# zabaras/deep-turbulence

Measured on AMD Instinct MI355X. Metric: flow-field samples/sec (fwd+log-det+bwd), 64x256x256x4; optimizer step: HipAdam (one-launch Adam, same update as torch.optim.Adam), higher is better.
Workload: dtype f32; 1 GPU; tmglow M: sample()+logdet+backward+Adam, out 256x256x4, L=4, K=16, batch 64/GPU; global_batch=64, parallelism=dp1, world_size_observed=1, rank0_device=AMD Radeon Graphics cuda:0, mix_precision=f32, launch=eager

## Files before the change

### deep-turbulence_amd/csrc/tmg_wino.hip

```cpp
#include "tmg_common.h"
#include <stdlib.h>
#include <type_traits>

struct WinoP {
    TmgSeg in[TMG_MAX_IN_SEG];
    int nseg;
    int B, Hin, Win;
    int Cin, Cin_pad, Cout, Npad;
    const float* U;
    const float* bias;
    int relu_in, pad_rep;
    TmgOSeg out[TMG_MAX_OUT_SEG];
    int tiles_x, tiles_y, ntiles;
    int nchunks;
};

__global__ void wino_pack_kernel(const float* __restrict__ w, float* __restrict__ U, int Cout, int Cin, int K, int N, int Kpad, int Npad, int mode) {
    const size_t total = (size_t)Kpad * Npad;
    for (size_t i = blockIdx.x * (size_t)blockDim.x + threadIdx.x; i < total; i += (size_t)gridDim.x * blockDim.x) {
        const int c16 = i & 15;
        size_t r = i >> 4;
        const int n = r % Npad;
        const int kb = r / Npad;
        const int k = kb * 16 + c16;
        float g[3][3];
#pragma unroll
        for (int a = 0; a < 3; ++a)
#pragma unroll
            for (int b = 0; b < 3; ++b) {
                float v = 0.f;
                if (k < K && n < N) v = mode == 0 ? w[((size_t)n * Cin + k) * 9 + a * 3 + b] : w[((size_t)k * Cin + n) * 9 + (2 - a) * 3 + (2 - b)];
                g[a][b] = v;
            }
        float t[4][3];
#pragma unroll
        for (int b = 0; b < 3; ++b) {
            t[0][b] = g[0][b];
            t[1][b] = 0.5f * (g[0][b] + g[1][b] + g[2][b]);
            t[2][b] = 0.5f * (g[0][b] - g[1][b] + g[2][b]);
            t[3][b] = g[2][b];
        }
#pragma unroll
        for (int a = 0; a < 4; ++a) {
            const float u0 = t[a][0], u1 = 0.5f * (t[a][0] + t[a][1] + t[a][2]), u2 = 0.5f * (t[a][0] - t[a][1] + t[a][2]), u3 = t[a][2];
            const size_t plane = (size_t)Kpad * Npad;
            U[(size_t)(a * 4 + 0) * plane + i] = u0;
            U[(size_t)(a * 4 + 1) * plane + i] = u1;
            U[(size_t)(a * 4 + 2) * plane + i] = u2;
            U[(size_t)(a * 4 + 3) * plane + i] = u3;
        }
    }
}

extern "C" int tmg_conv_wino_pack(const void* w, void* U, int64_t Cout, int64_t Cin, int64_t mode, int64_t nvalid, hipStream_t st) {
    const int K = mode == 0 ? (int)Cin : (int)Cout;
    const int N = mode == 0 ? (int)Cout : (int)(nvalid > 0 && nvalid < Cin ? nvalid : Cin);
    const int Kpad = (K + 15) & ~15, Npad = (N + 15) & ~15;
    const size_t total = (size_t)Kpad * Npad;
    const int blocks = (int)((total + 255) / 256 < 2048 ? (total + 255) / 256 : 2048);
    hipLaunchKernelGGL(wino_pack_kernel, dim3(blocks), dim3(256), 0, st, (const float*)w, (float*)U, (int)Cout, (int)Cin, K, N, Kpad, Npad, (int)mode);
    TMG_CHECK_LAUNCH();
    return 0;
}

constexpr int NT = 512;
constexpr int TH = 8, TW = 16, PH = TH + 2, PW = TW + 2, PP = PH * PW;
constexpr int KC = 32, CS = KC + 8;
constexpr int RAWW = PP * CS;
constexpr int UPI = (PP * (KC / 4) + NT - 1) / NT;
constexpr int VS = KC + 8;
constexpr int VPL = 32 * VS;

#define TMG_WN_TILE(T_)                                                                                               \
    int t_ = (T_);                                                                                                    \
    const int tx_ = t_ % p.tiles_x; t_ /= p.tiles_x;                                                                  \
    const int ty_ = t_ % p.tiles_y;                                                                                   \
    const int b_ = t_ / p.tiles_y;
#define TMG_WN_CURSORS                                                                                                \
    const int G = gridDim.x;                                                                                          \
    const int nmine = (int)blockIdx.x < p.ntiles ? (p.ntiles - (int)blockIdx.x + G - 1) / G : 0;                      \
    const int nchunks = p.nchunks, nst = nmine * nchunks;
#define TMG_WN_PATCH_TABLE                                                                                            \
    const int pc4 = tid & 7, ppix0 = tid >> 3;                                                                        \
    unsigned pyx[UPI];                                                                                                \
    _Pragma("unroll") for (int u = 0; u < UPI; ++u) {                                                                 \
        const int pix = min(ppix0 + u * 64, PP - 1);                                                                  \
        const int py = pix / PW, px = pix - py * PW;                                                                  \
        pyx[u] = ((unsigned)py << 16) | (unsigned)px;                                                                 \
    }                                                                                                                 \
    float4 pv[UPI];
#define TMG_WN_COMMIT                                                                                                 \
    if (k >= -1 && k + 1 < nst) {                                                                                     \
        float* rb_ = lds + ((k + 1) & 1) * RAWW;                                                                      \
        _Pragma("unroll") for (int u = 0; u < UPI; ++u) {                                                             \
            if (ppix0 + u * 64 < PP) {                                                                                \
                float4 v = pv[u];                                                                                     \
                if (p.relu_in) v = tmg_relu4(v); \
                *reinterpret_cast<float4*>(rb_ + (ppix0 + u * 64) * CS + 4 * pc4) = v;                                \
            }                                                                                                         \
        }                                                                                                             \
    }
#define TMG_WN_ISSUE_HEAD                                                                                             \
    TMG_WN_TILE(ti)                                                                                                   \
    const int iy0 = ty_ * TH - 1, ix0 = tx_ * TW - 1;                                                                 \
    TMG_PICK_IN_CHANNEL(p, ci * KC + 4 * pc4, true, tmg_zero_page, tptr, tss)
#define TMG_WN_ISSUE_TAIL if (++ci == nchunks) { ci = 0; ti += G; }
#define TMG_WN_PIXEL(U_)                                                                                              \
    const int iy = iy0 + (int)(pyx[U_] >> 16), ix = ix0 + (int)(pyx[U_] & 0xffffu);                                   \
    const int iyc = min(max(iy, 0), p.Hin - 1), ixc = min(max(ix, 0), p.Win - 1);                                     \
    const bool oob = !p.pad_rep && (iy != iyc || ix != ixc);
#define TMG_WN_TBV const unsigned tbv = (unsigned)b_ * (unsigned)(p.Hin * p.Win);
#define TMG_WN_PXI (tbv + (unsigned)iyc * (unsigned)p.Win + (unsigned)ixc)
#define TMG_WN_DEAD(U_) (oob || ppix0 + U_ * 64 >= PP)
#define TMG_WN_ISSUE(LOAD_)                                                                                           \
    if (k + 2 < nst) {                                                                                                \
        TMG_WN_ISSUE_HEAD                                                                                             \
        TMG_WN_TBV                                                                                                    \
        _Pragma("unroll") for (int u = 0; u < UPI; ++u) {                                                             \
            TMG_WN_PIXEL(u)                                                                                           \
            const float* a_ = TMG_WN_DEAD(u) ? tmg_zero_page : tptr + (size_t)TMG_WN_PXI * (unsigned)tss;             \
            LOAD_(pv[u], a_)                                                                                          \
        }                                                                                                             \
        TMG_WN_ISSUE_TAIL                                                                                             \
    }
#define TMG_WN_LD(D_, A_) D_ = *reinterpret_cast<const float4*>(A_);
#define TMG_WN_LD_NT(D_, A_)                                                                                          \
    {                                                                                                                 \
        const f32x4 nt_ = __builtin_nontemporal_load(reinterpret_cast<const f32x4*>(A_));                             \
        D_ = make_float4(nt_[0], nt_[1], nt_[2], nt_[3]);                                                             \
    }
#define TMG_W4(OP, A_, B_) make_float4(A_.x OP B_.x, A_.y OP B_.y, A_.z OP B_.z, A_.w OP B_.w)
#define TMG_WN_Y_RESET                                                                                                \
    _Pragma("unroll") for (int o = 0; o < 4; ++o) _Pragma("unroll") for (int m = 0; m < 2; ++m)                       \
        _Pragma("unroll") for (int n = 0; n < NPW; ++n) Y[o][m][n] = bvr[n];
#define TMG_WN_BIAS_Y                                                                                                 \
    f32x4 bvr[NPW];                                                                                                   \
    _Pragma("unroll") for (int n = 0; n < NPW; ++n) {                                                                 \
        const int n0 = (ntile0 + n) * 16 + 4 * q;                                                                     \
        const float* bp = (p.bias != nullptr && ntile0 + n < ntt && n0 < p.Cout) ? p.bias + n0 : tmg_zero_page;       \
        const float4 b4 = *reinterpret_cast<const float4*>(bp);                                                       \
        bvr[n] = (f32x4){b4.x, b4.y, b4.z, b4.w};                                                                     \
    }                                                                                                                 \
    f32x4 Y[4][2][NPW];                                                                                               \
    TMG_WN_Y_RESET
#define TMG_WN_EPILOGUE(LI_, Q_, STORE_)                                                                              \
    {                                                                                                                 \
        _Pragma("unroll") for (int m = 0; m < 2; ++m) {                                                               \
            const int wt = 16 * m + LI_;                                                                              \
            const int oyb = ty_ * TH + 2 * (wt >> 3), oxb = tx_ * TW + 2 * (wt & 7);                                  \
            _Pragma("unroll") for (int n = 0; n < NPW; ++n) {                                                         \
                const int n0 = (ntile0 + n) * 16 + 4 * Q_;                                                            \
                if (ntile0 + n < ntt && n0 < p.Cout) {                                                                \
                    int nl = n0;                                                                                      \
                    TMG_PICK_OSEG(p.out, nl, optr, ostride, ooff)                                                     \
                    _Pragma("unroll") for (int o = 0; o < 4; ++o) {                                                   \
                        const int oy = oyb + (o >> 1), ox = oxb + (o & 1);                                            \
                        if (oy < p.Hin && ox < p.Win) {                                                               \
                            const unsigned opx = ((unsigned)b_ * (unsigned)p.Hin + (unsigned)oy) * (unsigned)p.Win + (unsigned)ox; \
                            STORE_(Y[o][m][n], optr + (size_t)opx * (unsigned)ostride + ooff + nl)                    \
                        }                                                                                             \
                    }                                                                                                 \
                }                                                                                                     \
            }                                                                                                         \
        }                                                                                                             \
        TMG_WN_Y_RESET                                                                                                \
        cm = 0; tm += G;                                                                                              \
// ... 735 lines not shown
            if (cm + 1 == nchunks) {
#pragma unroll
                for (int e = 0; e < 2; ++e)
#pragma unroll
                    for (int m = 0; m < 2; ++m)
#pragma unroll
                        for (int n = 0; n < NTN; ++n) {
                            *reinterpret_cast<float4*>(Mb + ((pos0 + e) * 32 + 16 * m + li) * NC + 16 * n + 4 * q) =
                                make_float4(acc[e][m][n][0], acc[e][m][n][1], acc[e][m][n][2], acc[e][m][n][3]);
                            acc[e][m][n] = (f32x4){0.f, 0.f, 0.f, 0.f};
                        }
                __syncthreads();
                TMG_WN_TILE(tm)
                static_assert(32 * QN <= NT, "one epilogue item per thread");
                for (int it = tid; it < 32 * QN; it += NT) {
                    const int wt = it / QN, c4 = it - wt * QN;
                    const int n0 = 4 * c4;
                    if (n0 >= p.Cout) continue;
                    const float* mp_ = Mb + wt * NC + n0;
                    float4 z[2][4];
#pragma unroll
                    for (int nu = 0; nu < 4; ++nu) {
                        const float4 m0 = *reinterpret_cast<const float4*>(mp_ + (0 * 4 + nu) * 32 * NC);
                        const float4 m1 = *reinterpret_cast<const float4*>(mp_ + (1 * 4 + nu) * 32 * NC);
                        const float4 m2 = *reinterpret_cast<const float4*>(mp_ + (2 * 4 + nu) * 32 * NC);
                        const float4 m3 = *reinterpret_cast<const float4*>(mp_ + (3 * 4 + nu) * 32 * NC);
                        z[0][nu] = make_float4(m0.x + m1.x + m2.x, m0.y + m1.y + m2.y, m0.z + m1.z + m2.z, m0.w + m1.w + m2.w);
                        z[1][nu] = make_float4(m1.x - m2.x - m3.x, m1.y - m2.y - m3.y, m1.z - m2.z - m3.z, m1.w - m2.w - m3.w);
                    }
                    const float4 bv = bvq;
                    int nl = n0;
                    TMG_PICK_OSEG(p.out, nl, optr, ostride, ooff)
#pragma unroll
                    for (int oy = 0; oy < 2; ++oy)
#pragma unroll
                        for (int ox = 0; ox < 2; ++ox) {
                            const float4 za = z[oy][0], zb = z[oy][1], zc = z[oy][2], zd = z[oy][3];
                            float4 y = ox == 0 ? make_float4(za.x + zb.x + zc.x, za.y + zb.y + zc.y, za.z + zb.z + zc.z, za.w + zb.w + zc.w)
                                               : make_float4(zb.x - zc.x - zd.x, zb.y - zc.y - zd.y, zb.z - zc.z - zd.z, zb.w - zc.w - zd.w);
                            y.x += bv.x; y.y += bv.y; y.z += bv.z; y.w += bv.w;
                            if (p.relu_out) y = tmg_relu4(y);
                            const int py = ty_ * TH + 2 * (wt >> 3) + oy, px = tx_ * TW + 2 * (wt & 7) + ox;
                            if (py < p.Hin && px < p.Win)
                                *reinterpret_cast<float4*>(optr + (size_t)(((unsigned)b_ * (unsigned)p.Hin + (unsigned)py) * (unsigned)p.Win + (unsigned)px) * (unsigned)ostride + ooff + nl) = y;
                        }
                }
                cm = 0; tm += G;
            } else {
                ++cm;
            }
        }
        __syncthreads();
    }
#undef TMG_WN_STAGE
#undef TMG_WN_LOADG
}

template <int NTN>
static int launch_wino_nn(const WinoNP& p, int G, hipStream_t st, int64_t* plan) {
    const size_t lds_bytes = (size_t)(2 * 180 * 40 + 16 * 32 * (NTN * 16 + (NTN < 3 ? 4 : 0))) * sizeof(float);
    if (plan) { fill_wino_fwd_plan(plan, 3, NTN, p, G, 1, lds_bytes); return 0; }
    TMG_LDS_OPTIN((&wino_nn_kernel<NTN>));
    TmgProf prof(TMG_PROF_WINO, 2.0 * p.B * p.Hin * p.Win * (double)p.Cout * p.Cin * 9, st);
    hipLaunchKernelGGL((wino_nn_kernel<NTN>), dim3(G), dim3(512), lds_bytes, st, p);
    TMG_CHECK_LAUNCH();
    return 0;
}

static int wino_narrow_impl(const void* const* in_ptrs, const int64_t* in_desc, int64_t nseg, const void* U, const void* bias,
                            void* const* out_ptrs, const int64_t* out_desc, int64_t nout, const int64_t* dims, hipStream_t st, int64_t* plan) {
    WinoNP p;
    const int rc = wino_fwd_setup(p, in_ptrs, in_desc, nseg, U, bias, out_ptrs, out_desc, nout, dims, 16, true);
    if (rc != 1) return rc;
    p.relu_out = (int)dims[7];
    const int G = tmg_persistent_grid(1, p.ntiles);
    switch (p.Npad >> 4) {
        case 1: return launch_wino_nn<1>(p, G, st, plan);
        case 2: return launch_wino_nn<2>(p, G, st, plan);
        default: return launch_wino_nn<3>(p, G, st, plan);
    }
}

extern "C" int tmg_conv_wino_narrow(const void* const* in_ptrs, const int64_t* in_desc, int64_t nseg, const void* U, const void* bias,
                                    void* const* out_ptrs, const int64_t* out_desc, int64_t nout, const int64_t* dims, hipStream_t st) {
    return wino_narrow_impl(in_ptrs, in_desc, nseg, U, bias, out_ptrs, out_desc, nout, dims, st, nullptr);
}

extern "C" int tmg_conv_wino_narrow_plan(const void* const* in_ptrs, const int64_t* in_desc, int64_t nseg, const void* U, const void* bias,
                                         void* const* out_ptrs, const int64_t* out_desc, int64_t nout, const int64_t* dims, hipStream_t st,
                                         int64_t* plan) {
    if (!plan) return -3;
    for (int i = 0; i < TMG_WINO_FWD_PLAN_N; ++i) plan[i] = -1;
    return wino_narrow_impl(in_ptrs, in_desc, nseg, U, bias, out_ptrs, out_desc, nout, dims, st, plan);
}

struct WinoWP {
    TmgSeg in[TMG_MAX_IN_SEG];
    int nseg;
    int B, Hin, Win;
    int Cin, Cout;
    int relu_in, pad_rep;
    const float* dy; int dy_stride, dy_off;
    float* ws;
    int want_bias;
    const long long* gtab;
    int bpg, dy_goff;
    int tiles_x, tiles_y, ntiles;
};

template <int CIT, int NCO, bool DB>
__global__ __launch_bounds__(512, 1) void wino_wgrad_kernel(WinoWP p) {
    extern __shared__ __attribute__((aligned(16))) float lds[];
// ... 420 lines not shown
```

### deep-turbulence_amd/tmg_hip.py

```python
import ctypes
import os
import weakref
import subprocess
import sys

import torch

_HERE = os.path.dirname(os.path.abspath(__file__))
LIB_PATH = os.path.join(_HERE, "libtmglow_hip.so")
CSRC = os.path.join(_HERE, "csrc")
SOURCES = ["tmg_conv.hip", "tmg_pointwise.hip", "tmg_physics.hip", "tmg_mix16.hip", "tmg_coupling.hip", "tmg_wino.hip", "tmg_thin.hip", "tmg_glue.hip", "tmg_ensemble.hip", "tmg_spectrum.hip", "tmg_scores.hip", "tmg_tspec.hip", "tmg_quant.hip", "tmg_gram.hip", "tmg_sfun.hip", "tmg_event.hip", "tmg_pdf.hip", "tmg_pod.hip", "tmg_phase.hip", "tmg_spod.hip", "tmg_budget.hip", "tmg_corr.hip", "tmg_flux.hip", "tmg_vortex.hip", "tmg_frank.hip", "tmg_xspec.hip", "tmg_lagr.hip"]
NO_PACKED_F32 = ["tmg_wino.hip", "tmg_conv.hip", "tmg_coupling.hip", "tmg_thin.hip", "tmg_mix16.hip", "tmg_spectrum.hip", "tmg_tspec.hip",
                 "tmg_pod.hip", "tmg_spod.hip", "tmg_xspec.hip"]
_lib = None

c_i64 = ctypes.c_int64
c_vp = ctypes.c_void_p

EXPORTS = [
    "tmg_conv_pack", "tmg_conv_pack_map", "tmg_conv_fwd", "tmg_conv_fwd_add", "tmg_affine_bwd_scaled", "tmg_c1_fwd_add", "tmg_conv_wgrad", "tmg_conv_wgrad_ws_floats", "tmg_conv_rep_border_fix", "tmg_conv_dgrad_direct",
    "tmg_affine_apply", "tmg_affine_apply_pass", "tmg_bn_finalize", "tmg_affine_bwd", "tmg_lstm_pointwise_fwd", "tmg_lstm_pointwise_bwd", "tmg_gauss_fwd",
    "tmg_gauss_bwd", "tmg_checker", "tmg_upsample_fwd", "tmg_upsample_bwd", "tmg_chan_reduce", "tmg_bn_bwd_apply",
    "tmg_phys_fwd", "tmg_phys_rms", "tmg_phys_bwd", "tmg_conv_wgrad_grouped", "tmg_conv_wgrad_grouped_ws_floats", "tmg_conv_pack_batched", "tmg_masked_add", "tmg_c1x2_fwd", "tmg_c1_fwd", "tmg_c1_bwd", "tmg_dense2_bwd", "tmg_dkappa", "tmg_prof_enable", "tmg_prof_collect", "tmg_mix_f16", "tmg_phys_bwd_dev", "tmg_coupling_fwd", "tmg_coupling_bwd",
    "tmg_conv_wino_pack", "tmg_conv_wino_fwd", "tmg_conv_wino_narrow", "tmg_conv_wino_wgrad", "tmg_conv_wino_wgrad_ws_floats", "tmg_mix_f32", "tmg_lu_fold_fwd", "tmg_lu_fold_bwd", "tmg_lu_fold_bwd_split", "tmg_level_finish", "tmg_conv_wgrad_thin_grouped", "tmg_mix_wgrad_grouped", "tmg_layer_planes", "tmg_conv_wino_wgrad_grouped", "tmg_conv_wino_wgrad_grouped_ws_floats", "tmg_adam_step", "tmg_chan_moments", "tmg_bn_finalize64", "tmg_mix_f32_affine_fwd", "tmg_mix_f32_affine_bwd", "tmg_conv_pack_many", "tmg_pad_halves", "tmg_coupling_fwd_halves", "tmg_coupling_bwd_halves", "tmg_fill_i64", "tmg_conv_wino_pack3", "tmg_conv_wino_fwd3", "tmg_mat_inverse", "tmg_gauss_sample", "tmg_reverse_loss_fwd", "tmg_reverse_loss_bwd", "tmg_sum_terms", "tmg_vec_sum", "tmg_level_pack", "tmg_spread2", "tmg_phys_fields", "tmg_phys_fields_bwd",
    "tmg_gauss_sample_keyed", "tmg_ens_accum", "tmg_ens_time_finalize", "tmg_ens_turb_accum", "tmg_ens_turb_finalize",
    "tmg_spec_rows", "tmg_spec_cols", "tmg_spec_accum", "tmg_spec_finalize",
    "tmg_ens_score_store", "tmg_ens_score_step",
]
PLAN_EXPORTS = ["tmg_conv_fwd_plan", "tmg_conv_wgrad_plan", "tmg_conv_rep_border_plan", "tmg_conv_wino_fwd_plan", "tmg_conv_wino_fwd3_plan",
                "tmg_conv_wino_narrow_plan", "tmg_conv_wino_wgrad_plan", "tmg_c1x2_fwd_plan", "tmg_c1_fwd_plan",
                "tmg_conv_wgrad_thin_grouped_plan", "tmg_mix_wgrad_grouped_plan"]
TSPEC_EXPORTS = ["tmg_tspec_store", "tmg_tspec_block", "tmg_tspec_finalize"]
QUANT_EXPORTS = ["tmg_ens_quant_step"]
GRAM_EXPORTS = ["tmg_ens_gram_plan", "tmg_ens_gram_step", "tmg_ens_gram_traj"]
SFUN_EXPORTS = ["tmg_ens_sfun_plan", "tmg_ens_sfun_step"]
EVENT_EXPORTS = ["tmg_ens_event_plan", "tmg_ens_event_count", "tmg_ens_event_step"]
PDF_EXPORTS = ["tmg_ens_pdf_plan", "tmg_ens_pdf_count"]
POD_EXPORTS = ["tmg_ens_pod_plan", "tmg_ens_pod_project"]
PHASE_EXPORTS = ["tmg_ens_phase_plan", "tmg_ens_phase_label", "tmg_ens_phase_accum"]
SPOD_EXPORTS = ["tmg_ens_spod_plan", "tmg_ens_spod_csd", "tmg_ens_spod_modes"]
LAYOUT_EXPORTS = ["tmg_layer_unplanes"]
BUDGET_EXPORTS = ["tmg_ens_budget_plan", "tmg_ens_budget_accum", "tmg_ens_budget_terms"]
CORR_EXPORTS = ["tmg_ens_corr_plan", "tmg_ens_corr_probe", "tmg_ens_corr_accum", "tmg_ens_corr_finalize"]
FLUX_EXPORTS = ["tmg_ens_flux_plan", "tmg_ens_flux_accum", "tmg_ens_flux_terms"]
LAGR_EXPORTS = ["tmg_ens_lagr_plan", "tmg_ens_lagr_advect", "tmg_ens_lagr_store", "tmg_ens_lagr_finalize"]
VORTEX_EXPORTS = ["tmg_ens_vortex_plan", "tmg_ens_vortex_classify", "tmg_ens_vortex_label", "tmg_ens_vortex_census"]
FRANK_EXPORTS = ["tmg_ens_frank_plan", "tmg_ens_frank_step"]
XSPEC_EXPORTS = ["tmg_ens_xspec_plan", "tmg_ens_xspec_prep", "tmg_ens_xspec_cols", "tmg_ens_xspec_accum"]
_P64 = ctypes.POINTER(ctypes.c_int64)
FLUX_ARGTYPES = {
    "tmg_ens_flux_plan": [_P64, _P64, _P64],
    "tmg_ens_flux_accum": [ctypes.c_void_p, _P64, ctypes.c_void_p, ctypes.c_void_p, ctypes.c_void_p, _P64, _P64, ctypes.c_void_p],
    "tmg_ens_flux_terms": [ctypes.c_void_p, ctypes.c_void_p, ctypes.POINTER(ctypes.c_void_p), ctypes.c_void_p, _P64, _P64, ctypes.c_void_p],
}
FRANK_ARGTYPES = {
    "tmg_ens_frank_plan": [_P64, _P64],
    "tmg_ens_frank_step": [ctypes.c_void_p, ctypes.c_void_p, ctypes.c_int64, ctypes.c_void_p, ctypes.c_void_p, ctypes.c_void_p, _P64,
                           ctypes.c_void_p],
}
XSPEC_ARGTYPES = {
    "tmg_ens_xspec_plan": [_P64, _P64],
    "tmg_ens_xspec_prep": [ctypes.c_void_p, _P64, ctypes.c_void_p, ctypes.c_void_p, ctypes.c_void_p, ctypes.c_void_p, ctypes.c_void_p,
                           ctypes.c_void_p, _P64, ctypes.c_void_p],
    "tmg_ens_xspec_cols": [ctypes.c_void_p, ctypes.c_void_p, ctypes.c_void_p, ctypes.c_void_p, ctypes.c_void_p, ctypes.c_void_p, _P64,
                           ctypes.POINTER(ctypes.c_float), ctypes.c_void_p],
    "tmg_ens_xspec_accum": [ctypes.c_void_p] * 10 + [_P64, ctypes.c_void_p],
}
RET_I64 = ("tmg_conv_wgrad_ws_floats", "tmg_conv_wgrad_grouped_ws_floats", "tmg_conv_wino_wgrad_ws_floats",
           "tmg_conv_wino_wgrad_grouped_ws_floats")


def build(force=False, verbose=False):
    from concurrent.futures import ThreadPoolExecutor
    inc = os.path.join(os.path.dirname(_HERE), "include")
    headers = [os.path.join(CSRC, "tmg_common.h"), os.path.join(CSRC, "tmg_symgram.h"), os.path.join(CSRC, "tmg_field.h"), os.path.join(CSRC, "tmg_dft.h"),
               os.path.join(inc, "tmglow_hip.h"), os.path.join(inc, "tmglow_hip_plan.h"),
               os.path.join(inc, "tmglow_hip_tspec.h"), os.path.join(inc, "tmglow_hip_quant.h"),
               os.path.join(inc, "tmglow_hip_gram.h"), os.path.join(inc, "tmglow_hip_sfun.h"),
               os.path.join(inc, "tmglow_hip_event.h"), os.path.join(inc, "tmglow_hip_pdf.h"), os.path.join(inc, "tmglow_hip_pod.h"),
               os.path.join(inc, "tmglow_hip_phase.h"), os.path.join(inc, "tmglow_hip_spod.h"), os.path.join(inc, "tmglow_hip_layout.h"),
               os.path.join(inc, "tmglow_hip_budget.h"), os.path.join(inc, "tmglow_hip_corr.h"), os.path.join(inc, "tmglow_hip_flux.h"),
               os.path.join(inc, "tmglow_hip_lagr.h"), os.path.join(inc, "tmglow_hip_vortex.h"),
               os.path.join(inc, "tmglow_hip_frank.h"), os.path.join(inc, "tmglow_hip_xspec.h")]
    hmt = max(os.path.getmtime(h) for h in headers)
    objdir = os.path.join(_HERE, "build")
    os.makedirs(objdir, exist_ok=True)
    hipcc = os.environ.get("HIPCC", "/opt/rocm/bin/hipcc")
    flags = ["--offload-arch=gfx950", "-O3", "-fPIC", "-std=c++17", "-Wno-unused-result", "-I", inc]
    jobs, objs, stamps = [], [], []
    for src in SOURCES:
        sp, ob = os.path.join(CSRC, src), os.path.join(objdir, src.replace(".hip", ".o"))
        objs.append(ob)
        extra = ["-Xclang", "-target-feature", "-Xclang", "-packed-fp32-ops"] if src in NO_PACKED_F32 else []
        line = " ".join(flags + extra)
        stamp = ob + ".flags"
        old = open(stamp).read() if os.path.exists(stamp) else None
        if force or old != line or not os.path.exists(ob) or os.path.getmtime(ob) < max(os.path.getmtime(sp), hmt):
            jobs.append([hipcc] + flags + extra + ["-c", sp, "-o", ob])
            stamps.append((stamp, line))
    if not jobs and os.path.exists(LIB_PATH) and all(os.path.getmtime(LIB_PATH) >= os.path.getmtime(o) for o in objs):
        return LIB_PATH

    def run(cmd):
        if verbose:
            print(" ".join(cmd), flush=True)
        r = subprocess.run(cmd, stderr=subprocess.PIPE, text=True)
        err = "\n".join(ln for ln in r.stderr.splitlines() if "'-packed-fp32-ops' is not a recognized feature" not in ln)
        if err.strip():
            print(err, file=sys.stderr, flush=True)
        if r.returncode != 0:
            raise subprocess.CalledProcessError(r.returncode, cmd)

    with ThreadPoolExecutor(max_workers=4) as ex:
        list(ex.map(run, jobs))
    for stamp, line in stamps:
        open(stamp, "w").write(line)
    run([hipcc, "--offload-arch=gfx950", "-shared", "-fPIC"] + objs + ["-o", LIB_PATH])
    return LIB_PATH


def lib():
    global _lib
    if _lib is None:
        if not os.path.exists(LIB_PATH):
            raise RuntimeError("libtmglow_hip.so is missing (%s): run `python -c 'import __graft_entry__ as g; g.build()'`. "
                               "There is no fallback path." % LIB_PATH)
        _lib = ctypes.CDLL(LIB_PATH)
        for name in EXPORTS:
            getattr(_lib, name).restype = c_i64 if name in RET_I64 else ctypes.c_int
        _lib.tmg_prof_name.restype = ctypes.c_char_p
        for name in PLAN_EXPORTS:
            getattr(_lib, name).restype = ctypes.c_int
            getattr(_lib, name).argtypes = PLAN_ARGTYPES[name]
        for name in TSPEC_EXPORTS + QUANT_EXPORTS + GRAM_EXPORTS + SFUN_EXPORTS + EVENT_EXPORTS + PDF_EXPORTS + POD_EXPORTS + PHASE_EXPORTS + SPOD_EXPORTS + LAYOUT_EXPORTS + BUDGET_EXPORTS + CORR_EXPORTS + LAGR_EXPORTS + VORTEX_EXPORTS:
            getattr(_lib, name).restype = ctypes.c_int
        for name in FLUX_EXPORTS:
            getattr(_lib, name).restype = ctypes.c_int
            getattr(_lib, name).argtypes = FLUX_ARGTYPES[name]
        for name in FRANK_EXPORTS:
            getattr(_lib, name).restype = ctypes.c_int
            getattr(_lib, name).argtypes = FRANK_ARGTYPES[name]
        for name in XSPEC_EXPORTS:
            getattr(_lib, name).restype = ctypes.c_int
            getattr(_lib, name).argtypes = XSPEC_ARGTYPES[name]
    return _lib


def prof_enable(on):
    lib().tmg_prof_enable(c_i64(int(on)))


def prof_kernel_id(name):
    l = lib()
    for k in range(64):
        if l.tmg_prof_name(c_i64(k)).decode() == name:
            return k
    raise KeyError(name)


def prof_collect():
    l = lib()
    nk = 64
    buf = (ctypes.c_double * (3 * nk))()
    n = l.tmg_prof_collect(buf, c_i64(nk))
    out = {}
    for k in range(n):
        if buf[3 * k] > 0:
            out[l.tmg_prof_name(c_i64(k)).decode()] = (int(buf[3 * k]), buf[3 * k + 1], buf[3 * k + 2])
    return out


def _stream():
    return c_vp(torch._C._cuda_getCurrentRawStream(torch._C._cuda_getDevice()))


def _chk(code, name):
    if code != 0:
        raise RuntimeError("%s failed with code %d" % (name, code))


def _ptr(t):
    return c_vp(t.data_ptr()) if t is not None else c_vp(0)


def check_act(t):
    if not (t.is_cuda and t.dtype == torch.float32):
        raise RuntimeError("TM-Glow HIP ops need fp32 tensors on a HIP device (got %s on %s); there is no CPU path"
                           % (t.dtype, t.device))


def seg(t):
# ... 177 lines not shown
def wino_narrow_eligible(Cin, Cout):
    return Cout <= 48 and Cout % 4 == 0 and Cin % 4 == 0 and Cin >= 64


def conv_wino_pack(w, mode=0, nvalid=0):
    Cout, Cin = w.shape[0], w.shape[1]
    assert w.shape[2] == 3 and w.shape[3] == 3
    w = w.contiguous()
    K, N = (Cin, Cout) if mode == 0 else (Cout, nvalid if 0 < nvalid < Cin else Cin)
    U = torch.empty(16 * ((K + 15) // 16 * 16) * ((N + 15) // 16 * 16), device=w.device, dtype=torch.float32)
    _chk(lib().tmg_conv_wino_pack(_ptr(w), _ptr(U), c_i64(Cout), c_i64(Cin), c_i64(mode), c_i64(nvalid), _stream()), "tmg_conv_wino_pack")
    return U


_WINO_PRECISION = ["bf16x3" if os.environ.get("TMG_WINO_BF3") else "f32"]


def set_winograd_precision(kind):
    if kind not in ("f32", "bf16x3"):
        raise ValueError("Winograd precision must be 'f32' or 'bf16x3', got %r" % (kind,))
    _WINO_PRECISION[0] = kind


def winograd_precision():
    return _WINO_PRECISION[0]


def conv_wino_pack3(w, mode=0, nvalid=0):
    Cout, Cin = w.shape[0], w.shape[1]
    assert w.shape[2] == 3 and w.shape[3] == 3
    w = w.contiguous()
    K, N = (Cin, Cout) if mode == 0 else (Cout, nvalid if 0 < nvalid < Cin else Cin)
    U = torch.empty(16 * ((K + 31) // 32 * 32) * ((N + 15) // 16 * 16) * 3, device=w.device, dtype=torch.int16)
    _chk(lib().tmg_conv_wino_pack3(_ptr(w), _ptr(U), c_i64(Cout), c_i64(Cin), c_i64(mode), c_i64(nvalid), _stream()), "tmg_conv_wino_pack3")
    return U


def _wino_fwd(name, inputs, U, Cout, outs, bias, *flags):
    if isinstance(outs, torch.Tensor):
        outs = [outs]
    B, Hin, Win, _ = inputs[0].shape
    ip, idesc, n_in = _segs(inputs)
    op, odesc, n_out = _segs(outs)
    Cin = sum(t.shape[3] for t in inputs)
    assert sum(t.shape[3] for t in outs) == Cout and outs[0].shape[1] == Hin and outs[0].shape[2] == Win
    return _launched(getattr(lib(), name)(ip, idesc, c_i64(n_in), _ptr(U), _ptr(bias), op, odesc, c_i64(n_out),
                                          _i64(B, Hin, Win, Cin, Cout, *flags), _stream()), name)


def conv_wino_fwd3(inputs, U, Cout, outs, bias=None, relu_in=False, pad_rep=False):
    return _wino_fwd("tmg_conv_wino_fwd3", inputs, U, Cout, outs, bias, relu_in, pad_rep)


def conv_wino_narrow(inputs, U, Cout, outs, bias=None, relu_in=False, pad_rep=False, relu_out=False):
    return _wino_fwd("tmg_conv_wino_narrow", inputs, U, Cout, outs, bias, relu_in, pad_rep, relu_out)


def conv_wino_fwd(inputs, U, Cout, outs, bias=None, relu_in=False, pad_rep=False):
    return _wino_fwd("tmg_conv_wino_fwd", inputs, U, Cout, outs, bias, relu_in, pad_rep)


def conv3x3_auto(inputs, weight, Cout, outs, bias=None, relu_in=False, pad_rep=False, relu_out=False, dgrad=False, nvalid=0):
    Cin = sum(t.shape[3] for t in inputs)
    mode = 1 if dgrad else 0
    if not relu_out and wino_eligible(Cin, Cout, 3, 1):
        if (_WINO_PRECISION[0] == "bf16x3"
                and conv_wino_fwd3(inputs, conv_wino_pack3(weight, mode, nvalid), Cout, outs, bias=bias, relu_in=relu_in, pad_rep=pad_rep)):
            return None
        if conv_wino_fwd(inputs, conv_wino_pack(weight, mode, nvalid), Cout, outs, bias=bias, relu_in=relu_in, pad_rep=pad_rep):
            return None
    if wino_narrow_eligible(Cin, Cout):
        if conv_wino_narrow(inputs, conv_wino_pack(weight, mode, nvalid), Cout, outs, bias=bias, relu_in=relu_in, pad_rep=pad_rep,
                            relu_out=relu_out):
            return None
    wpk = conv_pack(weight, mode, nvalid, (nvalid, 1 << 30, 0)) if (dgrad and nvalid) else conv_pack(weight, mode)
    conv_fwd(inputs, wpk, Cout, 3, 1, outs, bias=bias, relu_in=relu_in, pad_rep=pad_rep, relu_out=relu_out)
    return wpk


_WS = {}


def workspace(nfloats, device):
    if torch.cuda.is_current_stream_capturing():
        return torch.empty(max(int(nfloats), 1), device=device, dtype=torch.float32)
    key = (device.index, torch._C._cuda_getCurrentRawStream(torch._C._cuda_getDevice()))
    buf = _WS.get(key)
    if buf is None or buf.numel() < nfloats:
        buf = torch.empty(max(int(nfloats), 1 << 20), device=device, dtype=torch.float32)
        _WS[key] = buf
    return buf


_WINO_WGRAD_CIN_MIN = 32
_WINO_WGRAD_PIX_MIN = 1 << 20


def conv_wgrad(inputs, dy, dW, dbias, ksize, stride, kappa=None, in_scale=None, in_shift=None, relu_in=False, pad_rep=False,
               use_ws=True, cin_dst=0, cin_valid=0, ci_split=0, ci_off0=0, ci_off1=0):
    B, Hin, Win, _ = inputs[0].shape
    _, Hout, Wout, Cout = dy.shape
    ip, idesc, n_in = _segs(inputs)
    Cin = sum(t.shape[3] for t in inputs)
    if (ksize == 3 and stride == 1 and kappa is None and in_scale is None and use_ws and Cin >= 32
            and (Cout >= 128 or (Cout >= 32 and Cin >= _WINO_WGRAD_CIN_MIN and B * Hin * Win >= _WINO_WGRAD_PIX_MIN))
            and conv_wino_wgrad(inputs, dy, dW, dbias, relu_in, pad_rep, cin_dst, cin_valid, ci_split, ci_off0, ci_off1)):
        return
# ... 349 lines not shown
    return out


def conv_fwd_plan(inputs, Cout, ksize, stride, outs, bias=None, kappa=None, in_scale=None, in_shift=None, relu_in=False,
                  pad_rep=False, relu_out=False, accumulate=False, add=None):
    ip, idesc, n_in, di = _psegs(inputs)
    op, odesc, n_out, do = _psegs(outs)
    (B, Hin, Win), (_, Hout, Wout) = di[0][0], do[0][0]
    Cin = sum(x[3] for x in di)
    dims = _i64(B, Hin, Win, Hout, Wout, ksize, stride, Cin, Cout, relu_in, pad_rep, relu_out, accumulate)
    ad = _i64(_pseg(add)[2], 0) if add is not None else _i64(0, 0)
    return _plan_call("tmg_conv_fwd_plan", FWD_PLAN_FIELDS, ip, idesc, n_in, c_vp(16), _pp(bias), _pp(kappa), _pp(in_scale),
                      _pp(in_shift), _pp(add), ad, op, odesc, n_out, dims, None)


def conv_wgrad_plan(inputs, dy, ksize, stride, dbias=None, kappa=None, in_scale=None, in_shift=None, relu_in=False, pad_rep=False,
                    use_ws=True, cin_dst=0, cin_valid=0, ci_split=0, ci_off0=0, ci_off1=0, ngroups=1):
    ip, idesc, n_in, di = _psegs(inputs)
    (B, Hin, Win) = di[0][0]
    (_, Hout, Wout), dyp, dys, Cout = _pseg(dy)
    Cin = sum(x[3] for x in di)
    dims = _i64(B, Hin, Win, Hout, Wout, ksize, stride, Cin, Cout, relu_in, pad_rep, cin_dst, cin_valid, ci_split, ci_off0, ci_off1)
    need = lib().tmg_conv_wgrad_grouped_ws_floats(dims, c_i64(ngroups)) if ngroups > 1 else lib().tmg_conv_wgrad_ws_floats(dims)
    return _plan_call("tmg_conv_wgrad_plan", WGRAD_PLAN_FIELDS, ip, idesc, n_in, _pp(in_scale), _pp(in_shift), c_vp(dyp), _i64(dys, 0),
                      c_vp(16), _pp(dbias), _pp(kappa), c_vp(16 if use_ws else 0), c_i64(need if use_ws else 0), dims, None, c_i64(ngroups))


def conv_rep_border_plan(dy, outs):
    (B, H, W), dyp, dys, Cdy = _pseg(dy)
    op, odesc, n_out, do = _psegs(outs)
    Cx = sum(x[3] for x in do)
    return _plan_call("tmg_conv_rep_border_plan", BORDER_PLAN_FIELDS, c_vp(dyp), _i64(dys, 0), c_vp(16), c_vp(0), op, odesc, n_out,
                      _i64(B, H, W, Cdy, Cx), None)


def _wino_fwd_plan(name, inputs, Cout, outs, bias, *flags):
    ip, idesc, n_in, di = _psegs(inputs)
    op, odesc, n_out, do = _psegs(outs)
    (B, Hin, Win) = di[0][0]
    Cin = sum(x[3] for x in di)
    return _plan_call(name, WINO_FWD_PLAN_FIELDS, ip, idesc, n_in, c_vp(16), _pp(bias), op, odesc, n_out,
                      _i64(B, Hin, Win, Cin, Cout, *flags), None)


def conv_wino_fwd_plan(inputs, Cout, outs, bias=None, relu_in=False, pad_rep=False):
    return _wino_fwd_plan("tmg_conv_wino_fwd_plan", inputs, Cout, outs, bias, relu_in, pad_rep)


def conv_wino_fwd3_plan(inputs, Cout, outs, bias=None, relu_in=False, pad_rep=False):
    return _wino_fwd_plan("tmg_conv_wino_fwd3_plan", inputs, Cout, outs, bias, relu_in, pad_rep)


def conv_wino_narrow_plan(inputs, Cout, outs, bias=None, relu_in=False, pad_rep=False, relu_out=False):
    return _wino_fwd_plan("tmg_conv_wino_narrow_plan", inputs, Cout, outs, bias, relu_in, pad_rep, relu_out)


def conv_wino_wgrad_plan(inputs, dy, dbias=None, relu_in=False, pad_rep=False, cin_dst=0, cin_valid=0, ci_split=0, ci_off0=0, ci_off1=0,
                         ngroups=1, use_ws=True):
    ip, idesc, n_in, di = _psegs(inputs)
    (B, Hin, Win) = di[0][0]
    _, dyp, dys, Cout = _pseg(dy)
    Cin = sum(x[3] for x in di)
    wd = _i64(B, Hin, Win, Cin, Cout, relu_in, pad_rep, cin_dst, cin_valid, ci_split, ci_off0, ci_off1)
    need = lib().tmg_conv_wino_wgrad_grouped_ws_floats(wd, c_i64(ngroups)) if ngroups > 1 else lib().tmg_conv_wino_wgrad_ws_floats(wd)
    return _plan_call("tmg_conv_wino_wgrad_plan", WINO_WGRAD_PLAN_FIELDS, ip, idesc, n_in, c_vp(dyp), _i64(dys, 0), c_vp(16), _pp(dbias),
                      c_vp(16 if use_ws else 0), c_i64(need if use_ws else 0), wd, None, c_i64(ngroups))


def c1x2_fwd_plan(inputs, out, add1=None, add2=None, w_rows=0, w2_d1_row=0, w_split=0, w_gap=0, relu_in=True):
    ip, idesc, n_in, di = _psegs(inputs)
    (B, Hh, Ww) = di[0][0]
    Cin = sum(x[3] for x in di)
    _, op, ostr, _ = _pseg(out)
    d2 = lambda t: _i64(_pseg(t)[2], 0) if t is not None else _i64(0, 0)
    return _plan_call("tmg_c1x2_fwd_plan", C1X2_PLAN_FIELDS, ip, idesc, n_in, c_vp(16), c_vp(16), _pp(add1), d2(add1), _pp(add2), d2(add2),
                      c_vp(op), _i64(ostr, 0), _i64(B, Hh, Ww, Cin, relu_in, w_rows, w_split, w_gap, w2_d1_row), None)


def c1_fwd_plan(inputs, out, add=None, w_rows=0, fill4=False, w_split=0, w_gap=0, relu_in=True):
    ip, idesc, n_in, di = _psegs(inputs)
    (B, Hh, Ww) = di[0][0]
    Cin = sum(x[3] for x in di)
    _, op, ostr, _ = _pseg(out)
    ad = _i64(_pseg(add)[2], 0) if add is not None else _i64(0, 0)
    return _plan_call("tmg_c1_fwd_plan", C1_PLAN_FIELDS, ip, idesc, n_in, c_vp(16), _pp(add), ad, c_vp(op), _i64(ostr, 0),
                      _i64(B, Hh, Ww, Cin, relu_in, w_rows, fill4, w_split, w_gap), None)


def conv_wgrad_thin_grouped_plan(shape3, seg_channels, G, dy_addr, dy_stride, dyc, relu_in=True):
    B, Hh, Ww = shape3
    return _plan_call("tmg_conv_wgrad_thin_grouped_plan", THIN_PLAN_FIELDS, c_vp(16), c_i64(G), _i64(*seg_channels), c_i64(len(seg_channels)),
                      c_vp(int(dy_addr)), c_i64(dy_stride), c_vp(16), _i64(B, Hh, Ww, sum(seg_channels), relu_in, dyc), None)


def mix_wgrad_grouped_plan(npix, C, G, db=True):
    return _plan_call("tmg_mix_wgrad_grouped_plan", MIX_WGRAD_PLAN_FIELDS, c_vp(16), c_i64(G), c_vp(16), _pp(db), _i64(npix, C), None)


def conv_dgrad_direct(dy, w, dx, ksize, stride, accumulate=False):
    B, Hin, Win, Cin = dx.shape
    _, Hout, Wout, Cout = dy.shape
    _chk(lib().tmg_conv_dgrad_direct(_ptr(dy), _d2(dy), _ptr(w), _ptr(dx), _d2(dx),
                                     _i64(B, Hin, Win, Hout, Wout, Cin, Cout, ksize, stride, accumulate), _stream()),
         "tmg_conv_dgrad_direct")


# ... 942 lines not shown
```

Measured before the change: 1543 samples/s.

## Add half-height Winograd narrow conv kernel with two blocks per CU

Adds a 256-thread variant of the narrow Winograd forward kernel that uses 4-row output tiles, so the LDS footprint is small enough for two blocks to share a CU. It also doubles the grid cap, and the existing 512-thread kernel is replaced for wide-N cases (NTN 2 and 3) when the pixel count reaches 2^20. The aim is more waves in flight, to hide global and LDS latency in the main convolutions. The cost is a larger halo fraction per tile (6 patch rows for 4 output rows) and more redundant input loads. The threshold can be changed through an environment variable.

Result: no change. 1550 samples/s (median of 4 runs) (+0.5%).

```diff
diff --git a/deep-turbulence_amd/csrc/tmg_wino.hip b/deep-turbulence_amd/csrc/tmg_wino.hip
--- a/deep-turbulence_amd/csrc/tmg_wino.hip
+++ b/deep-turbulence_amd/csrc/tmg_wino.hip
@@ -68,6 +68,7 @@
 constexpr int KC = 32, CS = KC + 8;
 constexpr int RAWW = PP * CS;
 constexpr int UPI = (PP * (KC / 4) + NT - 1) / NT;
+constexpr int PXS = NT / 8;
 constexpr int VS = KC + 8;
 constexpr int VPL = 32 * VS;
 
@@ -84,7 +85,7 @@
     const int pc4 = tid & 7, ppix0 = tid >> 3;                                                                        \
     unsigned pyx[UPI];                                                                                                \
     _Pragma("unroll") for (int u = 0; u < UPI; ++u) {                                                                 \
-        const int pix = min(ppix0 + u * 64, PP - 1);                                                                  \
+        const int pix = min(ppix0 + u * PXS, PP - 1);                                                                  \
         const int py = pix / PW, px = pix - py * PW;                                                                  \
         pyx[u] = ((unsigned)py << 16) | (unsigned)px;                                                                 \
     }                                                                                                                 \
@@ -93,10 +94,10 @@
     if (k >= -1 && k + 1 < nst) {                                                                                     \
         float* rb_ = lds + ((k + 1) & 1) * RAWW;                                                                      \
         _Pragma("unroll") for (int u = 0; u < UPI; ++u) {                                                             \
-            if (ppix0 + u * 64 < PP) {                                                                                \
+            if (ppix0 + u * PXS < PP) {                                                                                \
                 float4 v = pv[u];                                                                                     \
                 if (p.relu_in) v = tmg_relu4(v); \
-                *reinterpret_cast<float4*>(rb_ + (ppix0 + u * 64) * CS + 4 * pc4) = v;                                \
+                *reinterpret_cast<float4*>(rb_ + (ppix0 + u * PXS) * CS + 4 * pc4) = v;                                \
             }                                                                                                         \
         }                                                                                                             \
     }
@@ -111,7 +112,7 @@
     const bool oob = !p.pad_rep && (iy != iyc || ix != ixc);
 #define TMG_WN_TBV const unsigned tbv = (unsigned)b_ * (unsigned)(p.Hin * p.Win);
 #define TMG_WN_PXI (tbv + (unsigned)iyc * (unsigned)p.Win + (unsigned)ixc)
-#define TMG_WN_DEAD(U_) (oob || ppix0 + U_ * 64 >= PP)
+#define TMG_WN_DEAD(U_) (oob || ppix0 + U_ * PXS >= PP)
 #define TMG_WN_ISSUE(LOAD_)                                                                                           \
     if (k + 2 < nst) {                                                                                                \
         TMG_WN_ISSUE_HEAD                                                                                             \
@@ -953,12 +954,199 @@
         }
         __syncthreads();
     }
+#undef TMG_WN_LOADG
+}
+
+constexpr int NT_H = 256;
+constexpr int TH_H = 4, PH_H = TH_H + 2, PP_H = PH_H * PW;
+constexpr int RAWW_H = PP_H * CS;
+constexpr int UPI_H = (PP_H * (KC / 4) + NT_H - 1) / NT_H;
+constexpr int PXS_H = NT_H / 8;
+constexpr int wino_half_nc(int ntn) { return ntn * 16 + 4; }
+constexpr size_t wino_half_lds(int ntn) { return (size_t)(2 * RAWW_H + 4 * 2 * 16 * wino_half_nc(ntn)) * sizeof(float); }
+
+template <int NTN>
+__global__ __launch_bounds__(NT_H, 2) void wino_nn_half_kernel(WinoNP p) {
+    constexpr int TH = TH_H, PP = PP_H, RAWW = RAWW_H, UPI = UPI_H, PXS = PXS_H;
+    extern __shared__ __attribute__((aligned(16))) float lds[];
+    constexpr int NC = wino_half_nc(NTN);
+    float* Xb = lds + 2 * RAWW;
+    const int tid = threadIdx.x, lane = tid & 63;
+    const int nu = __builtin_amdgcn_readfirstlane(tid >> 6);
+    const int li = lane & 15, q = lane >> 4;
+    const int KB = p.Cin_pad >> 4;
+    const size_t kb_stride = (size_t)p.Npad * 16, pos_stride = (size_t)KB * p.Npad * 16;
+    const unsigned boff = 4u * (unsigned)(li * 16 + 4 * q);
+    const __amdgpu_buffer_rsrc_t urs = tmg_make_rsrc(p.U, 16u * (unsigned)pos_stride * 4u);
+    const int ca = nu == 0 ? 0 : (nu == 2 ? 2 : 1), cb = nu == 0 ? 2 : (nu == 1 ? 2 : (nu == 2 ? 1 : 3));
+    const float sc = nu == 1 ? 1.f : -1.f;
+    const int offa = (2 * (li >> 3) * PW + 2 * (li & 7) + ca) * CS + 4 * q;
+    const int offb = (2 * (li >> 3) * PW + 2 * (li & 7) + cb) * CS + 4 * q;
+
+    TMG_WN_PATCH_TABLE
+    constexpr bool PXC = true;
+    unsigned pxo[UPI];
+    unsigned pzm = 0;
+
+    TMG_WN_CURSORS
+    int ci = 0, cm = 0;
+    int ti = blockIdx.x, tm = blockIdx.x;
+
+    f32x4 acc[4][NTN];
+#pragma unroll
+    for (int xi = 0; xi < 4; ++xi)
+#pragma unroll
+        for (int n = 0; n < NTN; ++n) acc[xi][n] = (f32x4){0.f, 0.f, 0.f, 0.f};
+    constexpr int RD = 2;
+    float4 bq[RD][4][NTN];
+    const int ngrp = 2 * nchunks;
+#define TMG_WH_LOADP(SLOT, XI, GI)                                                                                    \
+    {                                                                                                                 \
+        const int kb_ = min((GI), KB - 1);                                                                            \
+        const unsigned so_ = 4u * (unsigned)((size_t)(4 * (XI) + nu) * pos_stride + (size_t)kb_ * kb_stride);        \
+        _Pragma("unroll") for (int n = 0; n < NTN; ++n) bq[SLOT][XI][n] = tmg_bload4(urs, boff, so_ + 1024u * n);     \
+    }
+    if (nst > 0) {
+#pragma unroll
+        for (int d = 0; d < RD; ++d)
+#pragma unroll
+            for (int xi = 0; xi < 4; ++xi) TMG_WH_LOADP(d, xi, d)
+    }
+
+    constexpr int QN = NTN * 4;
+    constexpr int NIT = (32 * QN + NT_H - 1) / NT_H;
+    float4 bvq[NIT];
+#pragma unroll
+    for (int j = 0; j < NIT; ++j) {
+        const int it = tid + j * NT_H, n0 = 4 * (it % QN);
+        const float* bp = (p.bias != nullptr && it < 32 * QN && n0 < p.Cout) ? p.bias + n0 : tmg_zero_page;
+        bvq[j] = *reinterpret_cast<const float4*>(bp);
+    }
+
+    for (int k = -2; k < nst; ++k) {
+        TMG_WN_STAGE
+        if (k >= 0) {
+            const float* rbuf = lds + (k & 1) * RAWW;
+            int gn = 2 * cm + RD;
+            if (gn >= ngrp) gn -= ngrp;
+#pragma unroll
+            for (int g = 0; g < 2; ++g) {
+                float4 da[4], db[4], v_[4];
+#pragma unroll
+                for (int r = 0; r < 4; ++r) {
+                    da[r] = *reinterpret_cast<const float4*>(rbuf + offa + r * PW * CS + g * 16);
+                    db[r] = *reinterpret_cast<const float4*>(rbuf + offb + r * PW * CS + g * 16);
+                }
+#define TMG_WH_V(XI, RA, OP, RB)                                                                                      \
+                {                                                                                                     \
+                    const float4 ua = TMG_W4(OP, da[RA], da[RB]), ub = TMG_W4(OP, db[RA], db[RB]);                    \
+                    v_[XI] = make_float4(fmaf(ub.x, sc, ua.x), fmaf(ub.y, sc, ua.y), fmaf(ub.z, sc, ua.z), fmaf(ub.w, sc, ua.w)); \
+                }
+                TMG_WH_V(0, 0, -, 2) TMG_WH_V(1, 1, +, 2) TMG_WH_V(2, 2, -, 1) TMG_WH_V(3, 1, -, 3)
+#undef TMG_WH_V
+                __builtin_amdgcn_sched_barrier(0);
+#pragma unroll
+                for (int xi = 0; xi < 4; ++xi) {
+#define TMG_WH_MFMA(E)                                                                                                \
+                    _Pragma("unroll") for (int n = 0; n < NTN; ++n)                                                   \
+                        acc[xi][n] = __builtin_amdgcn_mfma_f32_16x16x4f32(bq[g][xi][n].E, v_[xi].E, acc[xi][n], 0, 0, 0);
+                    TMG_WH_MFMA(x) TMG_WH_MFMA(y) TMG_WH_MFMA(z) TMG_WH_MFMA(w)
+#undef TMG_WH_MFMA
+                    __builtin_amdgcn_sched_barrier(0);
+                    TMG_WH_LOADP(g, xi, gn)
+                    __builtin_amdgcn_sched_barrier(0);
+                }
+                if (++gn == ngrp) gn = 0;
+            }
+            if (cm + 1 == nchunks) {
+#pragma unroll
+                for (int n = 0; n < NTN; ++n) {
+                    const f32x4 z0 = acc[0][n] + acc[1][n] + acc[2][n], z1 = acc[1][n] - acc[2][n] - acc[3][n];
+                    *reinterpret_cast<float4*>(Xb + ((nu * 2 + 0) * 16 + li) * NC + 16 * n + 4 * q) = make_float4(z0[0], z0[1], z0[2], z0[3]);
+                    *reinterpret_cast<float4*>(Xb + ((nu * 2 + 1) * 16 + li) * NC + 16 * n + 4 * q) = make_float4(z1[0], z1[1], z1[2], z1[3]);
+#pragma unroll
+                    for (int xi = 0; xi < 4; ++xi) acc[xi][n] = (f32x4){0.f, 0.f, 0.f, 0.f};
+                }
+                __syncthreads();
+                TMG_WN_TILE(tm)
+#pragma unroll
+                for (int j = 0; j < NIT; ++j) {
+                    const int it = tid + j * NT_H;
+                    const int r = it / QN, c4 = it - r * QN;
+                    const int wt = r & 15, oy = r >> 4;
+                    const int n0 = 4 * c4;
+                    if (it >= 32 * QN || n0 >= p.Cout) continue;
+                    const float* xp_ = Xb + (oy * 16 + wt) * NC + n0;
+                    const float4 za = *reinterpret_cast<const float4*>(xp_ + 0 * 32 * NC);
+                    const float4 zb = *reinterpret_cast<const float4*>(xp_ + 1 * 32 * NC);
+                    const float4 zc = *reinterpret_cast<const float4*>(xp_ + 2 * 32 * NC);
+                    const float4 zd = *reinterpret_cast<const float4*>(xp_ + 3 * 32 * NC);
+                    const float4 bv = bvq[j];
+                    int nl = n0;
+                    TMG_PICK_OSEG(p.out, nl, optr, ostride, ooff)
+                    const int py = ty_ * TH + 2 * (wt >> 3) + oy;
+#pragma unroll
+                    for (int ox = 0; ox < 2; ++ox) {
+                        float4 y = ox == 0 ? make_float4(za.x + zb.x + zc.x, za.y + zb.y + zc.y, za.z + zb.z + zc.z, za.w + zb.w + zc.w)
+                                           : make_float4(zb.x - zc.x - zd.x, zb.y - zc.y - zd.y, zb.z - zc.z - zd.z, zb.w - zc.w - zd.w);
+                        y.x += bv.x; y.y += bv.y; y.z += bv.z; y.w += bv.w;
+                        if (p.relu_out) y = tmg_relu4(y);
+                        const int px = tx_ * TW + 2 * (wt & 7) + ox;
+                        if (py < p.Hin && px < p.Win)
+                            *reinterpret_cast<float4*>(optr + (size_t)(((unsigned)b_ * (unsigned)p.Hin + (unsigned)py) * (unsigned)p.Win + (unsigned)px) * (unsigned)ostride + ooff + nl) = y;
+                    }
+                }
+                cm = 0; tm += G;
+            } else {
+                ++cm;
+            }
+        }
+        __syncthreads();
+    }
+#undef TMG_WH_LOADP
+}
 #undef TMG_WN_STAGE
-#undef TMG_WN_LOADG
+
+static const int64_t g_wino_half_default[3] = {INT64_MAX, 1 << 20, 1 << 20};
+static std::atomic<int64_t> g_wino_half_min{-1};
+extern "C" int tmg_conv_wino_half_min(int64_t pixels) {
+    g_wino_half_min.store(pixels < 0 ? -1 : pixels);
+    return 0;
+}
+static inline int64_t wino_half_min(int ntn) {
+    const int64_t v = g_wino_half_min.load();
+    return v < 0 ? g_wino_half_default[ntn - 1] : v;
+}
+
+template <int NTN>
+static int launch_wino_nn_half(WinoNP p, hipStream_t st, int64_t* plan) {
+    p.tiles_y = (p.Hin + TH_H - 1) / TH_H;
+    p.ntiles = p.B * p.tiles_x * p.tiles_y;
+    const int cap = 2 * tmg_num_cus();
+    const int G = cap > p.ntiles ? p.ntiles : cap;
+    const size_t lds_bytes = wino_half_lds(NTN);
+    static_assert(2 * wino_half_lds(3) <= 160 * 1024, "two blocks per CU");
+    if (plan) { fill_wino_fwd_plan(plan, 3, NTN, p, G, 1, lds_bytes); return 0; }
+    TMG_LDS_OPTIN((&wino_nn_half_kernel<NTN>));
+    TmgProf prof(TMG_PROF_WINO, 2.0 * p.B * p.Hin * p.Win * (double)p.Cout * p.Cin * 9, st);
+    hipLaunchKernelGGL((wino_nn_half_kernel<NTN>), dim3(G), dim3(NT_H), lds_bytes, st, p);
+    TMG_CHECK_LAUNCH();
+    return 0;
+}
+
+extern "C" int tmg_conv_wino_half_occupancy(int64_t ntn) {
+    int nb = 0;
+    hipError_t e = hipErrorInvalidValue;
+    if (ntn == 1) e = hipOccupancyMaxActiveBlocksPerMultiprocessor(&nb, wino_nn_half_kernel<1>, NT_H, wino_half_lds(1));
+    else if (ntn == 2) e = hipOccupancyMaxActiveBlocksPerMultiprocessor(&nb, wino_nn_half_kernel<2>, NT_H, wino_half_lds(2));
+    else if (ntn == 3) e = hipOccupancyMaxActiveBlocksPerMultiprocessor(&nb, wino_nn_half_kernel<3>, NT_H, wino_half_lds(3));
+    else return -3;
+    return e == hipSuccess ? nb : -(int)e;
 }
 
 template <int NTN>
 static int launch_wino_nn(const WinoNP& p, int G, hipStream_t st, int64_t* plan) {
+    if ((int64_t)p.B * p.Hin * p.Win >= wino_half_min(NTN)) return launch_wino_nn_half<NTN>(p, st, plan);
     const size_t lds_bytes = (size_t)(2 * 180 * 40 + 16 * 32 * (NTN * 16 + (NTN < 3 ? 4 : 0))) * sizeof(float);
     if (plan) { fill_wino_fwd_plan(plan, 3, NTN, p, G, 1, lds_bytes); return 0; }
     TMG_LDS_OPTIN((&wino_nn_kernel<NTN>));
diff --git a/deep-turbulence_amd/tmg_hip.py b/deep-turbulence_amd/tmg_hip.py
--- a/deep-turbulence_amd/tmg_hip.py
+++ b/deep-turbulence_amd/tmg_hip.py
@@ -30,6 +30,7 @@
 PLAN_EXPORTS = ["tmg_conv_fwd_plan", "tmg_conv_wgrad_plan", "tmg_conv_rep_border_plan", "tmg_conv_wino_fwd_plan", "tmg_conv_wino_fwd3_plan",
                 "tmg_conv_wino_narrow_plan", "tmg_conv_wino_wgrad_plan", "tmg_c1x2_fwd_plan", "tmg_c1_fwd_plan",
                 "tmg_conv_wgrad_thin_grouped_plan", "tmg_mix_wgrad_grouped_plan"]
+WINO_HALF_EXPORTS = ["tmg_conv_wino_half_min", "tmg_conv_wino_half_occupancy"]
 TSPEC_EXPORTS = ["tmg_tspec_store", "tmg_tspec_block", "tmg_tspec_finalize"]
 QUANT_EXPORTS = ["tmg_ens_quant_step"]
 GRAM_EXPORTS = ["tmg_ens_gram_plan", "tmg_ens_gram_step", "tmg_ens_gram_traj"]
@@ -81,7 +82,8 @@
                os.path.join(inc, "tmglow_hip_phase.h"), os.path.join(inc, "tmglow_hip_spod.h"), os.path.join(inc, "tmglow_hip_layout.h"),
                os.path.join(inc, "tmglow_hip_budget.h"), os.path.join(inc, "tmglow_hip_corr.h"), os.path.join(inc, "tmglow_hip_flux.h"),
                os.path.join(inc, "tmglow_hip_lagr.h"), os.path.join(inc, "tmglow_hip_vortex.h"),
-               os.path.join(inc, "tmglow_hip_frank.h"), os.path.join(inc, "tmglow_hip_xspec.h")]
+               os.path.join(inc, "tmglow_hip_frank.h"), os.path.join(inc, "tmglow_hip_xspec.h"),
+               os.path.join(inc, "tmglow_hip_wino_half.h")]
     hmt = max(os.path.getmtime(h) for h in headers)
     objdir = os.path.join(_HERE, "build")
     os.makedirs(objdir, exist_ok=True)
@@ -137,6 +139,9 @@
         for name in FLUX_EXPORTS:
             getattr(_lib, name).restype = ctypes.c_int
             getattr(_lib, name).argtypes = FLUX_ARGTYPES[name]
+        for name in WINO_HALF_EXPORTS:
+            getattr(_lib, name).restype = ctypes.c_int
+            getattr(_lib, name).argtypes = [c_i64]
         for name in FRANK_EXPORTS:
             getattr(_lib, name).restype = ctypes.c_int
             getattr(_lib, name).argtypes = FRANK_ARGTYPES[name]
@@ -420,7 +425,19 @@
     return _wino_fwd("tmg_conv_wino_fwd3", inputs, U, Cout, outs, bias, relu_in, pad_rep)
 
 
+def _wino_half_min():
+    v = os.environ.get("TMG_WINO_HALF_MIN", "")
+    lib().tmg_conv_wino_half_min(c_i64(int(v) if v != "" else -1))
+
+
+def wino_half_occupancy(ntn):
+    nb = int(lib().tmg_conv_wino_half_occupancy(c_i64(ntn)))
+    _chk(min(nb, 0), "tmg_conv_wino_half_occupancy")
+    return nb
+
+
 def conv_wino_narrow(inputs, U, Cout, outs, bias=None, relu_in=False, pad_rep=False, relu_out=False):
+    _wino_half_min()
     return _wino_fwd("tmg_conv_wino_narrow", inputs, U, Cout, outs, bias, relu_in, pad_rep, relu_out)
 
 
@@ -876,6 +893,7 @@
 
 
 def conv_wino_narrow_plan(inputs, Cout, outs, bias=None, relu_in=False, pad_rep=False, relu_out=False):
+    _wino_half_min()
     return _wino_fwd_plan("tmg_conv_wino_narrow_plan", inputs, Cout, outs, bias, relu_in, pad_rep, relu_out)
 
 
diff --git a/include/tmglow_hip_wino_half.h b/include/tmglow_hip_wino_half.h
--- /dev/null
+++ b/include/tmglow_hip_wino_half.h
@@ -0,0 +1,17 @@
+#ifndef TMGLOW_HIP_WINO_HALF_H
+#define TMGLOW_HIP_WINO_HALF_H
+
+#include "tmglow_hip.h"
+
+#ifdef __cplusplus
+extern "C" {
+#endif
+
+int tmg_conv_wino_half_min(int64_t pixels);
+
+int tmg_conv_wino_half_occupancy(int64_t ntn);
+
+#ifdef __cplusplus
+}
+#endif
+#endif
```
